# jason-li-831202/Vehicle-CV-ADAS

Measured on AMD Instinct MI355X. Metric: frames/sec end-to-end (detect+lane+NMS+track) per GPU; conv MFMA util %, higher is better.
Workload: dtype fp16x3

## Files before the change

### include/adas_hip.h

```cpp
#ifndef ADAS_HIP_H
#define ADAS_HIP_H
#include <stddef.h>
#include <stdint.h>

#ifdef __cplusplus
extern "C" {
#endif

typedef enum {
    ADAS_OK = 0,
    ADAS_ERR_INVALID = -1,
    ADAS_ERR_IO = -2,
    ADAS_ERR_FORMAT = -3,
    ADAS_ERR_HIP = -4,
    ADAS_ERR_CAPACITY = -5,
    ADAS_ERR_NO_DEVICE = -6
} adas_status;

const char* adas_last_error(void);
int adas_version(void);
int adas_device_count(void);
int adas_set_device(int index);
int adas_device_pci_bus_id(int index, char* out, int out_len);
int adas_malloc(void** d_ptr, size_t bytes);
// ... 5 lines not shown
int adas_host_free(void* h_ptr);
typedef struct adas_timer adas_timer;
int adas_timer_create(adas_timer** out);
int adas_timer_destroy(adas_timer* t);
int adas_timer_start(adas_timer* t, void* stream);
int adas_timer_stop(adas_timer* t, void* stream);
int adas_timer_elapsed_ms(adas_timer* t, float* ms);

typedef struct adas_engine adas_engine;

#define ADAS_PREC_BF16 0
#define ADAS_PREC_FP32 1
#define ADAS_PREC_FP16 2
#define ADAS_PREC_FP16X3 3

int adas_engine_create(const char* model_path, int precision, int max_batch, adas_engine** out);
int adas_engine_destroy(adas_engine* e);
int adas_engine_input_shape(const adas_engine* e, int64_t dims[4]);
int adas_engine_num_outputs(const adas_engine* e);
int adas_engine_output_shape(const adas_engine* e, int index, int64_t dims[4], int* ndim);
const char* adas_engine_output_name(const adas_engine* e, int index);
int adas_engine_infer_host(adas_engine* e, const float* h_input_nchw, int batch, float* const* h_outputs);
int adas_engine_infer_device(adas_engine* e, const float* d_input_nchw, int batch, void* stream);
int adas_engine_accepts_packed_input(const adas_engine* e);
int adas_engine_precision(const adas_engine* e);
int adas_engine_model_io_half(const adas_engine* e);
int adas_engine_infer_device_packed(adas_engine* e, const uint16_t* d_input_nhwc4, int batch, void* stream);
const float* adas_engine_output_device(const adas_engine* e, int index);
int adas_engine_stats(const adas_engine* e, double* flops_per_frame, double* weight_bytes, int* num_layers);
int adas_engine_profile(adas_engine* e, const float* d_input_nchw, int batch, int iters, float* ms_per_layer,
                        int max_layers, int* num_layers);
int adas_engine_detect_sink_supported(const adas_engine* e);
int adas_engine_detect_sink_shape(const adas_engine* e, int32_t* layout, int32_t* num_anchors, int32_t* num_classes);
int adas_engine_set_detect_sink(adas_engine* e, float* d_best_conf, int32_t* d_best_cls);
int adas_engine_layer_info(const adas_engine* e, int layer, char* name, int name_cap, double* flops, int* kind);
int adas_engine_layer_kernel(const adas_engine* e, int layer, int batch, char* name, int name_cap);
int adas_engine_prepare(adas_engine* e, int batch);
int adas_engine_ml_info(const adas_engine* e, int batch, int32_t* n_launches, int32_t* n_layers, int32_t* n_items);
int adas_engine_ml_status(const adas_engine* e, int batch, uint32_t* error_word);
int adas_engine_launch_count(adas_engine* e, int batch);
int adas_engine_ml_counters(const adas_engine* e, int batch, int launch, uint32_t head16[16]);
typedef struct adas_ml_view {
    uint64_t buf;
    int32_t cs, coff, c, h, w;
} adas_ml_view;
typedef struct adas_ml_layer_desc {
    int32_t kernel, stride, act, res_mode, up_c, halo_bn;
    adas_ml_view x, y, res, up;
} adas_ml_layer_desc;
int adas_debug_ml_plan(const adas_ml_layer_desc* layers, int n_layers, int batch, int precision, int32_t* deps, int32_t* targets,
                       uint64_t* items, int items_cap, int32_t summary[4]);
int adas_debug_conv_route(const adas_ml_layer_desc* layer, int batch, int precision, char* name, int name_cap);
int adas_debug_h8x3_onepass(const adas_ml_layer_desc* layer, int batch);
#define ADAS_PLAN_COLS 29
int adas_engine_plan(const adas_engine* e, int64_t* rows, int rows_cap, int32_t* n_ops, uint64_t* weight_bytes);
int adas_debug_engine_plan(const void* tables, size_t bytes, int precision, int max_batch, int64_t* rows, int rows_cap, int32_t* n_ops,
                           uint64_t* weight_bytes);
#define ADAS_LABEL_CAP 96
int adas_engine_schedule(const adas_engine* e, int batch, int32_t* step_of, int32_t* role, int cap, int32_t* n_ops, int32_t* n_steps);
int adas_debug_engine_schedule(const void* tables, size_t bytes, int precision, int max_batch, int batch, int32_t* step_of, int32_t* role,
                               char* labels, int cap, int32_t* n_ops, int32_t* n_steps);
int adas_engine_fetch_activation(adas_engine* e, int layer, int batch, float* h_out_nchw, int64_t dims[4]);

int adas_preprocess_yolo(const uint8_t* d_frames_bgr, int n, int src_h, int src_w, float* d_out_nchw, int dst_h,
                         int dst_w, int keep_ratio, void* stream);
int adas_preprocess_ufld(const uint8_t* d_frames_bgr, int n, int src_h, int src_w, float* d_out_nchw, int in_h,
                         int in_w, double crop_ratio, void* stream);
int adas_preprocess_yolo_packed(const uint8_t* d_frames_bgr, int n, int src_h, int src_w, uint16_t* d_out_nhwc4, int dst_h,
                                int dst_w, int keep_ratio, void* stream);
int adas_preprocess_ufld_packed(const uint8_t* d_frames_bgr, int n, int src_h, int src_w, uint16_t* d_out_nhwc4, int in_h,
                                int in_w, double crop_ratio, void* stream);
int adas_preprocess_yolo_packed_prec(const uint8_t* d_frames_bgr, int n, int src_h, int src_w, uint16_t* d_out_nhwc4, int dst_h,
                                     int dst_w, int keep_ratio, int precision, void* stream);
int adas_preprocess_ufld_packed_prec(const uint8_t* d_frames_bgr, int n, int src_h, int src_w, uint16_t* d_out_nhwc4, int in_h,
                                     int in_w, double crop_ratio, int precision, void* stream);

typedef struct adas_yolo_post adas_yolo_post;

#define ADAS_HEAD_V8 0
#define ADAS_HEAD_V5 1
#define ADAS_HEAD_V5_LITE 2
#define ADAS_NMS_REFERENCE 0
#define ADAS_NMS_GREEDY 1

typedef struct {
    int32_t layout;
    int32_t num_anchors;
    int32_t num_classes;
    int32_t nms_mode;
    double box_score;
    double iou_thr;
    int32_t pad_h, pad_w;
    double ratio_h, ratio_w;
    int32_t max_candidates;
    int32_t reserved;
} adas_yolo_post_params;

int adas_letterbox_params(int src_h, int src_w, int dst_h, int dst_w, int keep_ratio, adas_yolo_post_params* p);

int adas_yolo_post_create(const adas_yolo_post_params* p, int max_batch, adas_yolo_post** out);
int adas_yolo_post_destroy(adas_yolo_post* h);
int adas_yolo_post_set_input_size(adas_yolo_post* h, int in_h, int in_w);
int adas_yolo_post_run(adas_yolo_post* h, const float* d_head, int batch, void* stream);
int adas_yolo_post_scan_views(adas_yolo_post* h, float** d_best_conf, int32_t** d_best_cls);
int adas_yolo_post_run_prescanned(adas_yolo_post* h, const float* d_head, int batch, void* stream);
int adas_yolo_post_profile(adas_yolo_post* h, const float* d_head, int batch, int iters, float ms[2]);
// ... 490 lines not shown
```

### vehicle-cv-adas_amd/_lib.py

```python
import ctypes as C
import os

import numpy as np

HERE = os.path.dirname(os.path.abspath(__file__))
LIB_PATH = os.environ.get("ADAS_LIB") or os.path.join(HERE, "libadas_hip.so")

UFLD_MAX_POINTS = 128
HEAD_V8, HEAD_V5, HEAD_V5_LITE = 0, 1, 2
NMS_REFERENCE, NMS_GREEDY = 0, 1
PREC_BF16, PREC_FP32, PREC_FP16, PREC_FP16X3 = 0, 1, 2, 3
PRECISIONS = {"bf16": PREC_BF16, "fp32": PREC_FP32, "fp16": PREC_FP16, "fp16x3": PREC_FP16X3}


class AdasError(RuntimeError):
    def __init__(self, code, msg):
        super().__init__(f"libadas_hip error {code}: {msg}")
        self.code = code


class YoloPostParams(C.Structure):
    _fields_ = [("layout", C.c_int32), ("num_anchors", C.c_int32), ("num_classes", C.c_int32), ("nms_mode", C.c_int32),
                ("box_score", C.c_double), ("iou_thr", C.c_double), ("pad_h", C.c_int32), ("pad_w", C.c_int32),
                ("ratio_h", C.c_double), ("ratio_w", C.c_double), ("max_candidates", C.c_int32), ("reserved", C.c_int32)]
# ... 167 lines not shown


class MlView(C.Structure):
    _fields_ = [("buf", C.c_uint64), ("cs", C.c_int32), ("coff", C.c_int32), ("c", C.c_int32), ("h", C.c_int32), ("w", C.c_int32)]


class MlLayerDesc(C.Structure):
    _fields_ = [("kernel", C.c_int32), ("stride", C.c_int32), ("act", C.c_int32), ("res_mode", C.c_int32), ("up_c", C.c_int32), ("halo_bn", C.c_int32),
                ("x", MlView), ("y", MlView), ("res", MlView), ("up", MlView)]


TRACK_DTYPE = np.dtype([("tlwh", "f8", 4), ("score", "f8"), ("track_id", "i4"), ("state", "i4"), ("is_activated", "i4"),
                        ("class_id", "i4"), ("frame_id", "i4"), ("start_frame", "i4"), ("tracklet_len", "i4"), ("traj_len", "i4")])
TRAJECTORY_LEN = 30

_P = C.c_void_p
_SIGS = {
    "adas_last_error": (C.c_char_p, []),
    "adas_version": (C.c_int, []),
    "adas_device_count": (C.c_int, []),
    "adas_set_device": (C.c_int, [C.c_int]),
    "adas_device_pci_bus_id": (C.c_int, [C.c_int, C.c_char_p, C.c_int]),
    "adas_malloc": (C.c_int, [C.POINTER(_P), C.c_size_t]),
    "adas_free": (C.c_int, [_P]),
    "adas_memcpy_h2d": (C.c_int, [_P, _P, C.c_size_t]),
    "adas_memcpy_d2h": (C.c_int, [_P, _P, C.c_size_t]),
    "adas_synchronize": (C.c_int, []),
    "adas_host_alloc": (C.c_int, [C.POINTER(_P), C.c_size_t]),
    "adas_host_free": (C.c_int, [_P]),
    "adas_timer_create": (C.c_int, [C.POINTER(_P)]),
    "adas_timer_destroy": (C.c_int, [_P]),
    "adas_timer_start": (C.c_int, [_P, _P]),
    "adas_timer_stop": (C.c_int, [_P, _P]),
    "adas_timer_elapsed_ms": (C.c_int, [_P, C.POINTER(C.c_float)]),
    "adas_engine_create": (C.c_int, [C.c_char_p, C.c_int, C.c_int, C.POINTER(_P)]),
    "adas_engine_destroy": (C.c_int, [_P]),
    "adas_engine_input_shape": (C.c_int, [_P, C.POINTER(C.c_int64)]),
    "adas_engine_num_outputs": (C.c_int, [_P]),
    "adas_engine_output_shape": (C.c_int, [_P, C.c_int, C.POINTER(C.c_int64), C.POINTER(C.c_int)]),
    "adas_engine_output_name": (C.c_char_p, [_P, C.c_int]),
    "adas_engine_infer_host": (C.c_int, [_P, _P, C.c_int, C.POINTER(_P)]),
    "adas_engine_infer_device": (C.c_int, [_P, _P, C.c_int, _P]),
    "adas_engine_accepts_packed_input": (C.c_int, [_P]),
    "adas_engine_precision": (C.c_int, [_P]),
    "adas_engine_prepare": (C.c_int, [_P, C.c_int]),
    "adas_engine_ml_info": (C.c_int, [_P, C.c_int, C.POINTER(C.c_int32), C.POINTER(C.c_int32), C.POINTER(C.c_int32)]),
    "adas_engine_ml_status": (C.c_int, [_P, C.c_int, C.POINTER(C.c_uint32)]),
    "adas_engine_launch_count": (C.c_int, [_P, C.c_int]),
    "adas_engine_ml_counters": (C.c_int, [_P, C.c_int, C.c_int, C.POINTER(C.c_uint32)]),
    "adas_debug_ml_plan": (C.c_int, [C.POINTER(MlLayerDesc), C.c_int, C.c_int, C.c_int, C.POINTER(C.c_int32), C.POINTER(C.c_int32), C.POINTER(C.c_uint64),
                                     C.c_int, C.POINTER(C.c_int32)]),
    "adas_debug_conv_route": (C.c_int, [C.POINTER(MlLayerDesc), C.c_int, C.c_int, C.c_char_p, C.c_int]),
    "adas_debug_h8x3_onepass": (C.c_int, [C.POINTER(MlLayerDesc), C.c_int]),
    "adas_engine_plan": (C.c_int, [_P, C.POINTER(C.c_int64), C.c_int, C.POINTER(C.c_int32), C.POINTER(C.c_uint64)]),
    "adas_debug_engine_plan": (C.c_int, [C.c_char_p, C.c_size_t, C.c_int, C.c_int, C.POINTER(C.c_int64), C.c_int, C.POINTER(C.c_int32), C.POINTER(C.c_uint64)]),
    "adas_engine_schedule": (C.c_int, [_P, C.c_int, C.POINTER(C.c_int32), C.POINTER(C.c_int32), C.c_int, C.POINTER(C.c_int32), C.POINTER(C.c_int32)]),
    "adas_debug_engine_schedule": (C.c_int, [C.c_char_p, C.c_size_t, C.c_int, C.c_int, C.c_int, C.POINTER(C.c_int32), C.POINTER(C.c_int32), C.c_char_p,
                                             C.c_int, C.POINTER(C.c_int32), C.POINTER(C.c_int32)]),
    "adas_engine_model_io_half": (C.c_int, [_P]),
    "adas_engine_infer_device_packed": (C.c_int, [_P, _P, C.c_int, _P]),
    "adas_engine_output_device": (_P, [_P, C.c_int]),
    "adas_engine_stats": (C.c_int, [_P, C.POINTER(C.c_double), C.POINTER(C.c_double), C.POINTER(C.c_int)]),
    "adas_engine_profile": (C.c_int, [_P, _P, C.c_int, C.c_int, _P, C.c_int, C.POINTER(C.c_int)]),
    "adas_engine_layer_info": (C.c_int, [_P, C.c_int, C.c_char_p, C.c_int, C.POINTER(C.c_double), C.POINTER(C.c_int)]),
    "adas_engine_layer_kernel": (C.c_int, [_P, C.c_int, C.c_int, C.c_char_p, C.c_int]),
    "adas_engine_fetch_activation": (C.c_int, [_P, C.c_int, C.c_int, _P, C.POINTER(C.c_int64)]),
    "adas_preprocess_yolo": (C.c_int, [_P, C.c_int, C.c_int, C.c_int, _P, C.c_int, C.c_int, C.c_int, _P]),
    "adas_preprocess_ufld": (C.c_int, [_P, C.c_int, C.c_int, C.c_int, _P, C.c_int, C.c_int, C.c_double, _P]),
    "adas_preprocess_yolo_packed": (C.c_int, [_P, C.c_int, C.c_int, C.c_int, _P, C.c_int, C.c_int, C.c_int, _P]),
    "adas_preprocess_ufld_packed": (C.c_int, [_P, C.c_int, C.c_int, C.c_int, _P, C.c_int, C.c_int, C.c_double, _P]),
    "adas_preprocess_yolo_packed_prec": (C.c_int, [_P, C.c_int, C.c_int, C.c_int, _P, C.c_int, C.c_int, C.c_int, C.c_int, _P]),
    "adas_preprocess_ufld_packed_prec": (C.c_int, [_P, C.c_int, C.c_int, C.c_int, _P, C.c_int, C.c_int, C.c_double, C.c_int, _P]),
    "adas_letterbox_params": (C.c_int, [C.c_int, C.c_int, C.c_int, C.c_int, C.c_int, C.POINTER(YoloPostParams)]),
    "adas_yolo_post_create": (C.c_int, [C.POINTER(YoloPostParams), C.c_int, C.POINTER(_P)]),
    "adas_yolo_post_destroy": (C.c_int, [_P]),
    "adas_yolo_post_set_input_size": (C.c_int, [_P, C.c_int, C.c_int]),
    "adas_yolo_post_run": (C.c_int, [_P, _P, C.c_int, _P]),
    "adas_yolo_post_profile": (C.c_int, [_P, _P, C.c_int, C.c_int, C.POINTER(C.c_float)]),
    "adas_yolo_post_fetch": (C.c_int, [_P, C.c_int, C.POINTER(YoloCounts)] + [_P] * 9),
    "adas_yolo_post_fetch_dets": (C.c_int, [_P, C.c_int, C.POINTER(YoloCounts)] + [_P] * 5),
    "adas_yolo_post_device_views": (C.c_int, [_P] + [C.POINTER(_P)] * 4),
    "adas_yolo_post_scan_views": (C.c_int, [_P, C.POINTER(_P), C.POINTER(_P)]),
    "adas_yolo_post_run_prescanned": (C.c_int, [_P, _P, C.c_int, _P]),
    "adas_engine_detect_sink_supported": (C.c_int, [_P]),
    "adas_engine_detect_sink_shape": (C.c_int, [_P, C.POINTER(C.c_int32), C.POINTER(C.c_int32), C.POINTER(C.c_int32)]),
    "adas_engine_set_detect_sink": (C.c_int, [_P, _P, _P]),
    "adas_pipeline_detect_sink": (C.c_int, [_P]),
    "adas_yolo_post_capacity": (C.c_int, [_P, C.POINTER(C.c_int)]),
    "adas_yolo_post_head_shape": (C.c_int, [_P, C.POINTER(C.c_int32), C.POINTER(C.c_int32), C.POINTER(C.c_int32)]),
    "adas_effdet_post_create": (C.c_int, [C.POINTER(EffdetPostParams), C.c_int, C.POINTER(_P)]),
    "adas_effdet_post_destroy": (C.c_int, [_P]),
    "adas_effdet_post_run": (C.c_int, [_P, _P, _P, _P, _P, C.c_int, _P]),
    "adas_effdet_post_fetch": (C.c_int, [_P, C.c_int, C.POINTER(C.c_int32), _P, _P, _P, _P]),
    "adas_effdet_tail_create": (C.c_int, [C.POINTER(EffdetTailParams), C.c_int, C.POINTER(_P)]),
    "adas_effdet_tail_destroy": (C.c_int, [_P]),
    "adas_effdet_tail_run": (C.c_int, [_P, _P, _P, C.c_int, _P]),
    "adas_effdet_tail_fetch": (C.c_int, [_P, C.c_int, C.POINTER(C.c_int32), _P, _P, _P, C.POINTER(C.c_int32)]),
    "adas_effdet_tail_device_views": (C.c_int, [_P, C.POINTER(_P), C.POINTER(_P), C.POINTER(_P), C.POINTER(_P)]),
    "adas_preprocess_effdet": (C.c_int, [_P, C.c_int, C.c_int, C.c_int, _P, C.c_int, C.c_int, C.c_int, _P]),
    "adas_ufld_decode_create": (C.c_int, [C.POINTER(UfldParams), C.c_int, C.POINTER(_P)]),
    "adas_ufld_decode_destroy": (C.c_int, [_P]),
    "adas_ufld_decode_run": (C.c_int, [_P, _P, _P, _P, _P, C.c_size_t, C.c_size_t, C.c_size_t, C.c_size_t, C.c_int, _P]),
    "adas_ufld_decode_fetch": (C.c_int, [_P, C.c_int, _P, _P, _P]),
    "adas_ufld_decode_upload": (C.c_int, [_P, C.c_int, _P, _P, _P]),
    "adas_ufld1_decode_create": (C.c_int, [C.POINTER(Ufld1Params), C.c_int, C.POINTER(_P)]),
    "adas_ufld1_decode_set_source_size": (C.c_int, [_P, C.c_int, C.c_int]),
# ... 229 lines not shown
```

### vehicle-cv-adas_amd/csrc/conv_pw_x3.hip

```cpp
#include "kernels.h"
#include "elem16.h"
#include <stdlib.h>

namespace adas {

typedef __attribute__((ext_vector_type(4))) float wf32x4;
typedef __attribute__((ext_vector_type(4))) uint32_t wu32x4;

__device__ __forceinline__ float pwx_act(float v, int act) {
    if (act == ACT_SILU) return x3_silu(v);
    if (act == ACT_RELU) return fmaxf(v, 0.0f);
    if (act == ACT_LEAKY) return fmaxf(v, 0.1f * v);
    return v;
}

__device__ __forceinline__ void pwx_store(void* out, size_t o, const float v[4], int out_f32) {
    if (out_f32) *reinterpret_cast<float4*>((float*)out + o) = make_float4(v[0], v[1], v[2], v[3]);
    else x3_store4((x3s*)out + o, v);
}

struct PwxDev {
    const x3s* in;
    const uint16_t* wfrag;
    const float* bias;
    void* out;
    int in_cs, in_coff, cin;
    int out_cs, out_coff, cout, out_f32;
    int M;
    int stride, Wo, HoWo, W, HW;
    int act;
    int NT, NTL, mtiles;
    const x3s* up;
    int up_cs, up_coff, up_ks, up_W, up_HW;
};

template <int KS, bool TAIL>
__global__ __launch_bounds__(512) void conv_pwx3_kernel(PwxDev a) {
    Fp16::enter();
    extern __shared__ __attribute__((aligned(16))) uint16_t wl[];
    const int tid = threadIdx.x, lane = tid & 63, wave = tid >> 6;
    const int lrow = lane & 15, kg = lane >> 4;
    const int nt0 = blockIdx.y * a.NTL;
    const int ntl = a.NT - nt0 < a.NTL ? a.NT - nt0 : a.NTL;
    float* bl = reinterpret_cast<float*>(wl + (size_t)a.NTL * KS * 1024);
    {
        const int n16 = ntl * KS * 128;
        const uint16_t* wsrc = a.wfrag + (size_t)nt0 * KS * 1024;
        stage_lds16<512, 8>(wl, wsrc, n16, tid);
        for (int i = tid; i < ntl * 16; i += 512) bl[i] = a.bias[nt0 * 16 + i];
    }
    __syncthreads();
    const int tail_valid = a.cin - (KS - 1) * 32;
    const bool tail_zero = TAIL && kg * 8 >= tail_valid;

    for (int mt = blockIdx.x * 8 + wave; mt < a.mtiles; mt += gridDim.x * 8) {
        const int m = mt * 16 + lrow;
        const bool ok = m < a.M;
        const int mm = ok ? m : 0;
        size_t ipix;
        if (a.stride == 1) {
            ipix = (size_t)mm;
        } else {
            const int n = mm / a.HoWo, rem = mm - n * a.HoWo;
            const int oy = rem / a.Wo, ox = rem - oy * a.Wo;
            ipix = (size_t)n * a.HW + (size_t)(oy * a.stride) * a.W + ox * a.stride;
        }
        const wu32x4* ip = reinterpret_cast<const wu32x4*>(a.in + ipix * a.in_cs + a.in_coff + kg * 8);
        wu32x4 xh[KS], xl[KS];
        if (a.up) {
            const int n = mm / a.HW, rem = mm - n * a.HW;
            const int oy = rem / a.W, ox = rem - oy * a.W;
            const wu32x4* up = reinterpret_cast<const wu32x4*>(a.up + ((size_t)n * a.up_HW + (size_t)(oy >> 1) * a.up_W + (ox >> 1)) * a.up_cs + a.up_coff + kg * 8);
#pragma unroll
            for (int ks = 0; ks < KS; ++ks) {
                if (ks < a.up_ks) {
                    xh[ks] = up[ks * 8];
                    xl[ks] = up[ks * 8 + 1];
                } else {
                    xh[ks] = __builtin_nontemporal_load(ip + ks * 8);
                    xl[ks] = __builtin_nontemporal_load(ip + ks * 8 + 1);
                }
            }
        } else {
#pragma unroll
            for (int ks = 0; ks < KS; ++ks) {
                xh[ks] = __builtin_nontemporal_load(ip + ks * 8);
                xl[ks] = __builtin_nontemporal_load(ip + ks * 8 + 1);
            }
        }
        if (tail_zero) {
            xh[KS - 1] = wu32x4{0u, 0u, 0u, 0u};
            xl[KS - 1] = wu32x4{0u, 0u, 0u, 0u};
        }

        const size_t obase = (size_t)mm * a.out_cs + a.out_coff + kg * 4 + nt0 * 16;
        for (int nt = 0; nt < ntl; ++nt) {
            wf32x4 accm{0.f, 0.f, 0.f, 0.f}, accx{0.f, 0.f, 0.f, 0.f};
#pragma unroll
            for (int ks = 0; ks < KS; ++ks) {
                const uint16_t* wp = wl + ((size_t)(nt * KS + ks) * 128 + lane) * 8;
                const wu32x4 wh = *reinterpret_cast<const wu32x4*>(wp);
                const wu32x4 wlo = *reinterpret_cast<const wu32x4*>(wp + 512);
                accm = Fp16::mfma(wh, xh[ks], accm);
                accx = Fp16::mfma(wh, xl[ks], accx);
                accx = Fp16::mfma(wlo, xh[ks], accx);
            }
            const int c = nt * 16 + kg * 4;
            if (!ok || nt0 * 16 + c >= a.cout) continue;
            const float4 b4 = *reinterpret_cast<const float4*>(bl + c);
            const float bb[4] = {b4.x, b4.y, b4.z, b4.w};
            float v[4];
#pragma unroll
            for (int r = 0; r < 4; ++r) v[r] = pwx_act((accm[r] + accx[r] * kX3Down) + bb[r], a.act);
            pwx_store(a.out, obase + nt * 16, v, a.out_f32);
        }
    }
}

static const int PWX_MAX_LDS = 150 * 1024;

static int pwx_max_split() {
    static int v = -1;
    if (v < 0) {
        const char* e = getenv("ADAS_PWX3_MAXSPLIT");
        v = e ? atoi(e) : 4;
        if (v < 0) v = 0;
        if (v > 8) v = 8;
    }
    return v;
}
static int pwx_tiles_per_wg(int nt, int ks) {
    for (int split = 1; split <= pwx_max_split(); ++split) {
        const int ntl = (nt + split - 1) / split;
        if ((size_t)ntl * ks * 2048 + (size_t)ntl * 64 <= (size_t)PWX_MAX_LDS) return ntl;
    }
    return 0;
}

bool pw_x3_applicable(int kh, int kw, int stride, int pad, int res_mode, const TView& in, const TView& out) {
    if (in.f32) return false;
    if (kh != 1 || kw != 1 || pad != 0 || (stride != 1 && stride != 2) || res_mode != RES_NONE) return false;
    if (in.h == 1 && in.w == 1) return false;
    if ((in.c & 7) || (in.cs & 7) || (in.coff & 7) || (out.c & 3) || (out.cs & 3) || (out.coff & 3)) return false;
    if (!out.f32 && ((out.c & 7) || (out.cs & 7) || (out.coff & 7))) return false;
    const int ks = (in.c + 31) / 32, nt = (out.c + 15) / 16;
    if (!(ks <= 6 || ks == 8 || ks == 10 || ks == 12 || ks == 16)) return false;
    return pwx_tiles_per_wg(nt, ks) > 0;
}

template <int KS>
static hipError_t pwx_launch(const PwxDev& d, bool tail, dim3 grid, size_t lds, hipStream_t st) {
    static bool attr_done = false;
    if (!attr_done) {
        (void)hipFuncSetAttribute((const void*)conv_pwx3_kernel<KS, false>, hipFuncAttributeMaxDynamicSharedMemorySize, PWX_MAX_LDS);
        (void)hipFuncSetAttribute((const void*)conv_pwx3_kernel<KS, true>, hipFuncAttributeMaxDynamicSharedMemorySize, PWX_MAX_LDS);
        attr_done = true;
    }
    if (tail) hipLaunchKernelGGL((conv_pwx3_kernel<KS, true>), grid, dim3(512), lds, st, d);
    else hipLaunchKernelGGL((conv_pwx3_kernel<KS, false>), grid, dim3(512), lds, st, d);
    return hipGetLastError();
}

hipError_t launch_conv_pw_x3(const ConvArgs& a, hipStream_t st) {
    PwxDev d;
    d.in = (const x3s*)a.in.p; d.wfrag = (const uint16_t*)a.wgt; d.bias = a.bias; d.out = a.out.p;
    d.in_cs = a.in.cs; d.in_coff = a.in.coff; d.cin = a.in.c;
    d.out_cs = a.out.cs; d.out_coff = a.out.coff; d.cout = a.out.c; d.out_f32 = a.out.f32;
    d.M = a.m; d.stride = a.stride; d.Wo = a.out.w; d.HoWo = a.out.h * a.out.w; d.W = a.in.w; d.HW = a.in.h * a.in.w;
    d.act = a.act;
    d.up = nullptr; d.up_cs = d.up_coff = d.up_ks = d.up_W = d.up_HW = 0;
    if (a.up_c > 0) {
        if (a.stride != 1 || (a.up_c & 31) || a.up.c != a.up_c || 2 * a.up.h != a.in.h || 2 * a.up.w != a.in.w || a.up.f32 || ((a.up.cs | a.up.coff) & 7)) return hipErrorInvalidValue;
        d.up = (const x3s*)a.up.p; d.up_cs = a.up.cs; d.up_coff = a.up.coff; d.up_ks = a.up_c / 32; d.up_W = a.up.w; d.up_HW = a.up.h * a.up.w;
    }
    const int ks = (a.in.c + 31) / 32;
    d.NT = (a.out.c + 15) / 16;
    d.mtiles = (a.m + 15) / 16;
    d.NTL = pwx_tiles_per_wg(d.NT, ks);
    if (d.NTL <= 0) return hipErrorNotSupported;
    const int nsplit = (d.NT + d.NTL - 1) / d.NTL;
    const size_t lds = (size_t)d.NTL * ks * 2048 + (size_t)d.NTL * 64;
    int per_cu = (int)((160 * 1024) / (lds > 4096 ? lds : 4096));
    if (per_cu > 4) per_cu = 4;
    if (per_cu < 1) per_cu = 1;
    int gx = 256 * per_cu / nsplit;
    if (gx < 1) gx = 1;
    const int need = (d.mtiles + 7) / 8;
    if (gx > need) gx = need;
    const dim3 grid(gx, nsplit);
    const bool tail = (a.in.c & 31) != 0;
    switch (ks) {
        case 1: return pwx_launch<1>(d, tail, grid, lds, st);
        case 2: return pwx_launch<2>(d, tail, grid, lds, st);
        case 3: return pwx_launch<3>(d, tail, grid, lds, st);
        case 4: return pwx_launch<4>(d, tail, grid, lds, st);
        case 5: return pwx_launch<5>(d, tail, grid, lds, st);
        case 6: return pwx_launch<6>(d, tail, grid, lds, st);
        case 8: return pwx_launch<8>(d, tail, grid, lds, st);
        case 10: return pwx_launch<10>(d, tail, grid, lds, st);
        case 12: return pwx_launch<12>(d, tail, grid, lds, st);
        case 16: return pwx_launch<16>(d, tail, grid, lds, st);
    }
    return hipErrorInvalidValue;
}

struct FcxDev {
    const x3s* x;
    const uint16_t* w;
    const float* bias;
    void* out;
    int x_cs, x_coff, out_cs, out_coff;
    int batch, cout, kpad, act, out_f32;
};

template <int TN, int TM, int KS, int U>
__global__ __launch_bounds__(64 * KS) void fc_x3_kernel(FcxDev a) {
    Fp16::enter();
    const int tid = threadIdx.x, lane = tid & 63, wave = tid >> 6;
    const int lrow = lane & 15, kg = lane >> 4;
    const int n0 = blockIdx.x * (TN * 16);
    const int KT = a.kpad >> 5;
    const int ks0 = (int)((long)KT * wave / KS), ks1 = (int)((long)KT * (wave + 1) / KS);
    const int n = ks1 - ks0;

    const wu32x4* wp[TN];
#pragma unroll
    for (int i = 0; i < TN; ++i) wp[i] = reinterpret_cast<const wu32x4*>(a.w) + ((size_t)(blockIdx.x * TN + i) * KT + ks0) * 128 + lane;
    const wu32x4* xp[TM];
#pragma unroll
    for (int j = 0; j < TM; ++j) {
        const int m = j * 16 + lrow;
        xp[j] = reinterpret_cast<const wu32x4*>(a.x + (size_t)(m < a.batch ? m : 0) * a.x_cs + a.x_coff + kg * 8 + ks0 * 32);
    }

    wf32x4 accm[TN][TM], accx[TN][TM];
#pragma unroll
    for (int i = 0; i < TN; ++i)
#pragma unroll
        for (int j = 0; j < TM; ++j) {
            accm[i][j] = wf32x4{0.f, 0.f, 0.f, 0.f};
            accx[i][j] = wf32x4{0.f, 0.f, 0.f, 0.f};
        }
// ... 183 lines not shown
```

### vehicle-cv-adas_amd/csrc/engine.cpp

```cpp
#include "engine.h"
#include <string.h>
#include <string>
#include <vector>

using namespace adas;

int adas::free_engine(adas_engine* e) {
    if (!e) return ADAS_OK;
    for (auto& kv : e->schedules) free_schedule(&kv.second);
    e->schedules.clear();
    for (auto& b : e->bufs)
        if (b.d && b.alias_of < 0) (void)hipFree(b.d);
    if (e->d_weights) (void)hipFree(e->d_weights);
    if (e->d_input) (void)hipFree(e->d_input);
    for (auto& ev : e->events)
        if (ev) (void)hipEventDestroy(ev);
    delete e;
    return ADAS_OK;
}

extern "C" {

int adas_engine_destroy(adas_engine* e) { return free_engine(e); }

// ... 341 lines not shown
    a.k = a.kh * a.kw * a.in.c; a.kpad = (a.kh * a.kw * ((a.in.c + 31) / 32 * 32) + 31) / 32 * 32; a.m = batch * a.out.h * a.out.w; a.max_n = batch; a.prec = precision;
    a.halo_bn = d.halo_bn;
    if (d.up_c > 0) { a.up = view(d.up); a.up_c = d.up_c; }
    return a;
}

int adas_debug_ml_plan(const adas_ml_layer_desc* layers, int n_layers, int batch, int precision, int32_t* deps, int32_t* targets, uint64_t* items,
                       int items_cap, int32_t summary[4]) {
    ADAS_REQUIRE(layers && n_layers > 0 && batch > 0 && deps && targets && summary, ADAS_ERR_INVALID, "adas_debug_ml_plan: bad argument");
    std::vector<ConvArgs> ls;
    std::vector<int> ks;
    for (int i = 0; i < n_layers; ++i) {
        ls.push_back(conv_args_of_desc(layers[i], batch, precision));
        ks.push_back(layers[i].kernel);
    }
    std::string why;
    MlPlanInfo info;
    MlPlan* pl = ml_plan_create(ls, ks, precision, &why, &info, true);
    ADAS_REQUIRE(pl, ADAS_ERR_INVALID, "adas_debug_ml_plan: %s", why.c_str());
    ml_plan_destroy(pl);
    for (int i = 0; i < n_layers; ++i)
        for (int k = 0; k < ML_MAX_DEPS; ++k) {
            deps[i * ML_MAX_DEPS + k] = k < (int)info.deps[i].size() ? info.deps[i][k] : -1;
            targets[i * ML_MAX_DEPS + k] = k < (int)info.targets[i].size() ? info.targets[i][k] : 0;
        }
    summary[0] = info.n_items; summary[1] = info.grid; summary[2] = (int32_t)info.lds; summary[3] = info.order;
    if (items) {
        ADAS_REQUIRE(items_cap >= info.n_items, ADAS_ERR_CAPACITY, "adas_debug_ml_plan: %d items, room for %d", info.n_items, items_cap);
        for (int k = 0; k < info.n_items; ++k) items[k] = info.item_words[k];
    }
    return ADAS_OK;
}

int adas_debug_conv_route(const adas_ml_layer_desc* layer, int batch, int precision, char* name, int name_cap) {
    ADAS_REQUIRE(layer && batch > 0 && precision >= PREC_BF16 && precision <= PREC_X3 && name && name_cap > 0, ADAS_ERR_INVALID,
                 "adas_debug_conv_route: bad argument");
    ConvArgs a = conv_args_of_desc(*layer, batch, precision);
    const ConvPlan pl = plan_conv(precision, a.kh, a.kw, a.stride, a.pad, a.max_n, a.res_mode, a.in, a.out);
    a.kpad = pl.kpad;
    if (wants_x3h8_packing(precision, pl.kernel, a.kh, a.kw, a.stride, a.pad, a.res_mode, a.in, a.out)) a.wgt_h8x3 = (const void*)(uintptr_t)0x1000;
    snprintf(name, name_cap, "%s", conv_kernel_name(a));
    return ADAS_OK;
}

int adas_debug_h8x3_onepass(const adas_ml_layer_desc* layer, int batch) {
    if (!layer || batch <= 0) return -1;
    ConvArgs a = conv_args_of_desc(*layer, batch, PREC_X3);
    const ConvPlan pl = plan_conv(PREC_X3, a.kh, a.kw, a.stride, a.pad, a.max_n, a.res_mode, a.in, a.out);
    a.kpad = pl.kpad;
    if (wants_x3h8_packing(PREC_X3, pl.kernel, a.kh, a.kw, a.stride, a.pad, a.res_mode, a.in, a.out)) a.wgt_h8x3 = (const void*)(uintptr_t)0x1000;
    return (conv_route(a) == ConvRoute::H8X3 && halo8_x3_onepass(a)) ? 1 : 0;
}

int adas_engine_precision(const adas_engine* e) { return e ? e->prec : -1; }
int adas_engine_model_io_half(const adas_engine* e) { return e ? (int)((e->hdr.in_cpad >> 16) & 1u) : 0; }

int adas_engine_accepts_packed_input(const adas_engine* e) {
    return (e && e->prec != PREC_X3 && e->ops.size() >= 2 && e->ops[0].skip && e->ops[1].kernel == CONV_STEM) ? 1 : 0;
}

int adas_engine_infer_device_packed(adas_engine* e, const uint16_t* d_input_nhwc4, int batch, void* stream) {
    ADAS_REQUIRE(e && d_input_nhwc4 && batch > 0 && batch <= e->max_batch, ADAS_ERR_INVALID, "adas_engine_infer_device_packed: bad argument");
    ADAS_REQUIRE(adas_engine_accepts_packed_input(e), ADAS_ERR_INVALID,
                 "this engine's first layer is not the fused stem (fp32 mode or ADAS_NO_STEM): feed the fp32 NCHW tensor instead");
    e->last = (hipStream_t)stream;
    return engine_forward(e, reinterpret_cast<const float*>(d_input_nhwc4), batch, (hipStream_t)stream, true);
}

const float* adas_engine_output_device(const adas_engine* e, int index) {
    if (!e || index < 0 || index >= (int)e->outs.size()) return nullptr;
    const EngOut& o = e->outs[index];
    return (const float*)e->bufs[o.buf].d + o.offset;
}

int adas_engine_infer_host(adas_engine* e, const float* h_input, int batch, float* const* h_outputs) {
    ADAS_REQUIRE(e && h_input && h_outputs && batch > 0 && batch <= e->max_batch, ADAS_ERR_INVALID, "adas_engine_infer_host: bad argument");
    size_t in_bytes = (size_t)batch * e->hdr.in_c * e->hdr.in_h * e->hdr.in_w * 4;
    ADAS_HIP_TRY(hipMemcpyAsync(e->d_input, h_input, in_bytes, hipMemcpyHostToDevice, 0));
    int rc = adas_engine_infer_device(e, e->d_input, batch, nullptr);
    if (rc != ADAS_OK) return rc;
    for (size_t i = 0; i < e->outs.size(); ++i) {
        const EngOut& o = e->outs[i];
        const EngBuf& b = e->bufs[o.buf];
        size_t frame_stride = (size_t)b.h * b.w * b.c;
        ADAS_HIP_TRY(hipMemcpy2DAsync(h_outputs[i], o.elems * 4, (const float*)b.d + o.offset, frame_stride * 4, o.elems * 4, batch,
                                      hipMemcpyDeviceToHost, 0));
    }
    ADAS_HIP_TRY(hipStreamSynchronize(0));
    if (e->mode == adas_engine::ML) {
        uint32_t w = 0;
        int rc = adas_engine_ml_status(e, batch, &w);
        if (rc != ADAS_OK) return rc;
    }
    return ADAS_OK;
}

int adas_engine_profile(adas_engine* e, const float* d_input, int batch, int iters, float* ms_per_layer, int max_layers, int* num_layers) {
    ADAS_REQUIRE(e && d_input && batch > 0 && batch <= e->max_batch && iters > 0 && ms_per_layer, ADAS_ERR_INVALID, "adas_engine_profile: bad argument");
    const int n = (int)e->ops.size();
    ADAS_REQUIRE(max_layers >= n, ADAS_ERR_INVALID, "need room for %d layers", n);
    {
        int rc = engine_prepare(e, batch);
        if (rc != ADAS_OK) return rc;
    }
    const std::vector<Step>& steps = e->schedules.at(batch).steps;
    const size_t n_ev = (steps.size() > 8 ? steps.size() : 8) + 1;
// ... 71 lines not shown
```

### vehicle-cv-adas_amd/csrc/kernels.h

```cpp
#pragma once
#include <hip/hip_runtime.h>
#include <stdint.h>

namespace adas {

enum { PREC_BF16 = 0, PREC_FP32 = 1, PREC_FP16 = 2, PREC_X3 = 3 };
inline bool prec_is16(int prec) { return prec == PREC_BF16 || prec == PREC_FP16; }
inline int prec_esize(int prec) { return prec_is16(prec) ? 2 : 4; }
enum { ACT_NONE = 0, ACT_SILU = 1, ACT_RELU = 2, ACT_LEAKY = 3 ,
       ACT_HSWISH = 4 , ACT_HSIGMOID = 5 , ACT_RELU6 = 6  };
enum { RES_NONE = 0, RES_AFTER_ACT = 1, RES_BEFORE_ACT = 2 };

int persist_slots(int which);

struct TView {
    void* p;
    int cs, coff, c;
    int h, w;
    int f32;
};

struct ConvArgs {
    TView in, out, res;
    const void* wgt;
// ... 88 lines not shown
bool depth2space_supported(const TView& in, const TView& out);
hipError_t launch_depth2space(TView in, TView out, int n, int prec, hipStream_t st);
hipError_t launch_detect_v6(const TView* ins, float* out, int n, int nc, int A, const int strides[3], hipStream_t st);
hipError_t launch_detect_v6_dfl(const TView* ins, float* out, int n, int nc, int A, const int strides[3], hipStream_t st);
bool sppf_pool3_applicable(int prec, const TView& in, const TView out[3]);
hipError_t launch_sppf_pool3(const TView& in, const TView out[3], int n, int prec, hipStream_t st);
hipError_t launch_detect_v8(const TView* ins, float* out, int n, int nc, int A, const int strides[3], hipStream_t st);
hipError_t launch_detect_v8_fused(const TView* hidden, const void* const* wfrag, const float* const* bias, float* out, int n, int nc, int A,
                                  const int strides[3], int prec, hipStream_t st, float* sink_conf = nullptr, int* sink_cls = nullptr);
hipError_t launch_detect_v8_fused_x3(const TView* hidden, const void* const* wfrag, const float* const* bias, int kt_box, int kt_cls, float* out, int n, int nc,
                                     int A, const int strides[3], hipStream_t st_, float* sink_conf = nullptr, int* sink_cls = nullptr);
bool det5_applicable(int prec, int nc, const TView& in, const TView& logits);
size_t det5_weight_bytes(int no, int cin);
hipError_t launch_pack_weights_det5(const float* src, void* dst, int no, int cin, int prec, hipStream_t st);
hipError_t launch_detect_v5_fused(const TView* hidden, const void* const* wfrag, const float* const* bias, float* out, int n, int nc, int A,
                                  const int strides[3], const float* d_anchors, int prec, hipStream_t st, float* sink_conf = nullptr, int* sink_cls = nullptr);
hipError_t launch_detect_v5(const TView* ins, float* out, int n, int nc, int A, const int strides[3],
                            const float* d_anchors, hipStream_t st);
hipError_t launch_layernorm(const float* in, void* out, const float* gamma, const float* beta, int n, int len, float eps,
                            int prec, hipStream_t st);
hipError_t launch_pack_weights(const float* src, void* dst, int cout, int cout_pad, int taps, int cin, int cin_pad, int kpad,
                               int prec, hipStream_t st);
bool stem_applicable(int prec, int in_c_true, int kh, int kw, int stride, int pad, int act, int res_mode, const TView& out, bool pool,
                     const TView& pool_out);
size_t stem_weight_bytes(int kh, int cout);
size_t stem2_weight_bytes();
void stem2_pack_weights(const float* w_ohwi_32x3x3x16, uint16_t* dst_host, int prec);
bool stem2_applicable(int prec, int kh, int pad, int act, const TView& stem_out, int kh2, int kw2, int stride2, int pad2, int act2, int res_mode2,
                      const TView& out2);
hipError_t launch_conv_stem2(const float* nchw, int n, int c_true, int H, int W, int kh, int pad, const void* wfrag, const float* bias,
                             const TView& stem_out, const void* wfrag2, const float* bias2, const TView& out2, bool packed_in, int prec, hipStream_t st);
void stem_pack_weights(const float* w_ohwi, int cout, int kh, int kw, int cs, int c_true, uint16_t* dst_host, int prec);
bool stem_x3_applicable(int in_c_true, int kh, int kw, int stride, int pad, int act, int res_mode, const TView& out);
size_t stem_x3_weight_bytes(int kh, int cout);
void stem_x3_pack_weights(const float* w_ohwi, int cout, int kh, int kw, int cs, int c_true, uint16_t* dst_host);
hipError_t launch_conv_stem_x3(const float* nchw, int n, int c_true, int H, int W, int kh, int pad, int act, const void* wfrag, const float* bias,
                               const TView& out, hipStream_t st);
bool stem2_x3_applicable(int in_c_true, int kh, int pad, int act, const TView& stem_out, int kh2, int kw2, int stride2, int pad2, int act2, int res_mode2,
                         const TView& out2);
size_t stem2_x3_weight_bytes();
void stem2_x3_pack_weights(const float* w_ohwi_32x3x3x16, uint16_t* dst_host);
hipError_t launch_conv_stem2_x3(const float* nchw, int n, int c_true, int H, int W, int kh, int pad, const void* wfrag, const float* bias,
                                const TView& stem_out, const void* wfrag2, const float* bias2, const TView& out2, hipStream_t st);
bool stem_pool_x3_applicable(int in_c_true, int kh, int kw, int stride, int pad, int act, int res_mode, const TView& conv_out, const TView& pool_out);
hipError_t launch_conv_stem_pool_x3(const float* nchw, int n, int c_true, int H, int W, int pad, const void* wfrag, const float* bias,
                                    const TView& conv_out, const TView& pool_out, hipStream_t st);
hipError_t launch_conv_stem(const float* nchw, int n, int c_true, int H, int W, int kh, int pad, int act, const void* wfrag,
                            const float* bias, const TView& conv_out, bool pool, const TView& pool_out, bool packed_in, int prec, hipStream_t st);
inline int halo_bn(int cout) { return cout <= 16 ? 16 : (cout <= 32 ? 32 : ((cout > 64 && cout <= 96) ? 48 : 64)); }
int plan_halo_bn(int max_n, int stride, const TView& in, const TView& out);
hipError_t launch_pack_weights_halo(const float* src, void* dst, int cout, int cout_pad, int cin, int cin_pad, int prec, hipStream_t st, int bn = 0);
bool pw_x3_applicable(int kh, int kw, int stride, int pad, int res_mode, const TView& in, const TView& out);
hipError_t launch_conv_pw_x3(const ConvArgs& a, hipStream_t st);
bool fc_x3_applicable(int kh, int kw, int stride, const TView& in, const TView& out);
hipError_t launch_fc_x3(const ConvArgs& a, hipStream_t st);
hipError_t launch_pack_weights_fcx3(const float* src, void* dst, int cout, int cout_pad, int cin, int kpad, hipStream_t st);
hipError_t launch_pack_weights_fc(const float* src, void* dst, int cout, int cout_pad, int cin, int kpad, int prec, hipStream_t st);
bool se_gate_supported(const TView& in, const TView& gate, int cr, uint64_t w_elems, uint64_t b_elems);
hipError_t launch_se_gate(const TView& in, const TView& gate, const float* w1, const float* w2, int cr, int act_hidden, int act_gate, int n, int prec, hipStream_t st,
                          const TView* scratch = nullptr);
bool scale_supported(const TView& in, const TView& gate, const TView& out);
hipError_t launch_scale(const TView& in, const TView& gate, const TView& out, int n, int prec, hipStream_t st);
bool shuffle_supported(const TView& in, const TView& out, int groups);
hipError_t launch_shuffle(const TView& in, const TView& out, int groups, int n, int prec, hipStream_t st);
bool wsum_supported(int n_in, const TView* ins, const TView& out);
hipError_t launch_wsum(int n_in, const TView* ins, const float* w, const TView& out, int n, int act, int prec, hipStream_t st);
bool dwconv_supported(int k, int stride, int pad, int res_mode, const TView& in, const TView& out);
hipError_t launch_dwconv(const TView& in, const TView& out, const TView& res, int res_mode, const float* wgt, const float* bias, int n, int k,
                         int stride, int pad, int act, int prec, hipStream_t st);
bool attention_supported(int nh, int kd, int hd, const TView& qkv, const TView& out);
hipError_t launch_attention(const TView& qkv, const TView& out, int n, int nh, int kd, int hd, float scale, int prec, hipStream_t st);
hipError_t launch_nhwc_to_nchw(TView in, float* out, int n, int prec, hipStream_t st);

}
```

Measured before the change: 5660.

## Add K-streaming pointwise fp16x3 conv kernel with async LDS pipelining

Adds a new pointwise fp16x3 conv body that streams the K dimension. Activation and weight chunks are loaded with buffer_load_lds into a 2-3 slot ring buffer, and a persistent grid walks over M passes. The old body keeps all weights for a column split resident in LDS. The new body is chosen by default when that old plan would split the output channels or use more than 80KB of LDS and there are enough passes. The aim is to stop reloading activations once per output-channel split and to raise occupancy, at the cost of re-streaming weights for every pass and adding more barriers.

```diff
diff --git a/include/adas_hip.h b/include/adas_hip.h
--- a/include/adas_hip.h
+++ b/include/adas_hip.h
@@ -81,6 +81,8 @@
                        uint64_t* items, int items_cap, int32_t summary[4]);
 int adas_debug_conv_route(const adas_ml_layer_desc* layer, int batch, int precision, char* name, int name_cap);
 int adas_debug_h8x3_onepass(const adas_ml_layer_desc* layer, int batch);
+int adas_debug_pwx3_body(int mode);
+int adas_debug_pwx3_plan(int cin, int cout, int m, int stride, int out[4]);
 #define ADAS_PLAN_COLS 29
 int adas_engine_plan(const adas_engine* e, int64_t* rows, int rows_cap, int32_t* n_ops, uint64_t* weight_bytes);
 int adas_debug_engine_plan(const void* tables, size_t bytes, int precision, int max_batch, int64_t* rows, int rows_cap, int32_t* n_ops,
diff --git a/vehicle-cv-adas_amd/_lib.py b/vehicle-cv-adas_amd/_lib.py
--- a/vehicle-cv-adas_amd/_lib.py
+++ b/vehicle-cv-adas_amd/_lib.py
@@ -243,6 +243,8 @@
                                      C.c_int, C.POINTER(C.c_int32)]),
     "adas_debug_conv_route": (C.c_int, [C.POINTER(MlLayerDesc), C.c_int, C.c_int, C.c_char_p, C.c_int]),
     "adas_debug_h8x3_onepass": (C.c_int, [C.POINTER(MlLayerDesc), C.c_int]),
+    "adas_debug_pwx3_body": (C.c_int, [C.c_int]),
+    "adas_debug_pwx3_plan": (C.c_int, [C.c_int, C.c_int, C.c_int, C.c_int, C.POINTER(C.c_int)]),
     "adas_engine_plan": (C.c_int, [_P, C.POINTER(C.c_int64), C.c_int, C.POINTER(C.c_int32), C.POINTER(C.c_uint64)]),
     "adas_debug_engine_plan": (C.c_int, [C.c_char_p, C.c_size_t, C.c_int, C.c_int, C.POINTER(C.c_int64), C.c_int, C.POINTER(C.c_int32), C.POINTER(C.c_uint64)]),
     "adas_engine_schedule": (C.c_int, [_P, C.c_int, C.POINTER(C.c_int32), C.POINTER(C.c_int32), C.c_int, C.POINTER(C.c_int32), C.POINTER(C.c_int32)]),
diff --git a/vehicle-cv-adas_amd/csrc/conv_pw_x3.hip b/vehicle-cv-adas_amd/csrc/conv_pw_x3.hip
--- a/vehicle-cv-adas_amd/csrc/conv_pw_x3.hip
+++ b/vehicle-cv-adas_amd/csrc/conv_pw_x3.hip
@@ -1,6 +1,7 @@
 #include "kernels.h"
 #include "elem16.h"
 #include <stdlib.h>
+#include <atomic>
 
 namespace adas {
 
@@ -32,6 +33,8 @@
     int NT, NTL, mtiles;
     const x3s* up;
     int up_cs, up_coff, up_ks, up_W, up_HW;
+    uint32_t in_bytes, up_bytes, wgt_bytes;
+    int npass;
 };
 
 template <int KS, bool TAIL>
@@ -117,6 +120,169 @@
     }
 }
 
+constexpr uint32_t PWK_OOB = 0xF0000000u;
+constexpr int PWK_MIN_PASSES = 128;
+typedef __attribute__((address_space(3))) void* pwk_lds_vp;
+
+template <int N>
+__device__ __forceinline__ void pwk_wait_vm() {
+    asm volatile("s_waitcnt vmcnt(%0) lgkmcnt(0)" ::"n"(N) : "memory");
+}
+
+template <int NTG, int G>
+struct PwkGeom {
+    static constexpr int PT = 2, NPT = (8 / G) * PT;
+    static constexpr int ACT_B = NPT * 2048, WGT_B = G * NTG * 2048, SLOT = ACT_B + WGT_B, BIAS_B = 2048;
+    static constexpr int NS = 3 * SLOT + BIAS_B <= 160 * 1024 ? 3 : 2;
+    static constexpr int APW = NPT * 2 / 8, WPW = G * NTG * 2 / 8, PPW = APW + WPW;
+    static constexpr int LDS = NS * SLOT + BIAS_B;
+};
+
+template <int KS, int NTG, int G>
+__global__ __launch_bounds__(512) void conv_pwx3_kstream_kernel(PwxDev a) {
+    using Gm = PwkGeom<NTG, G>;
+    constexpr int PT = Gm::PT, NPT = Gm::NPT, NS = Gm::NS, APW = Gm::APW, WPW = Gm::WPW, SLOT = Gm::SLOT, ACT_B = Gm::ACT_B;
+    Fp16::enter();
+    extern __shared__ __attribute__((aligned(16))) uint16_t wl[];
+    unsigned char* lds8 = reinterpret_cast<unsigned char*>(wl);
+    const int tid = threadIdx.x, lane = tid & 63, wave = __builtin_amdgcn_readfirstlane(tid >> 6);
+    const int lrow = lane & 15, kg = lane >> 4;
+    const int g = wave % G, s = wave / G;
+    const int t0 = g * a.NTL;
+    const int nmine = a.NT - t0 < a.NTL ? (a.NT - t0 > 0 ? a.NT - t0 : 0) : a.NTL;
+    float* bl = reinterpret_cast<float*>(lds8 + NS * SLOT);
+    for (int i = tid; i < a.NT * 16; i += 512) bl[i] = a.bias[i];
+    __syncthreads();
+    const int tail_valid = a.cin - (KS - 1) * 32;
+    const bool tail_zero = kg * 8 >= tail_valid;
+
+    __amdgpu_buffer_rsrc_t rin = __builtin_amdgcn_make_buffer_rsrc((void*)a.in, 0, a.in_bytes, 0x00020000);
+    __amdgpu_buffer_rsrc_t rup = __builtin_amdgcn_make_buffer_rsrc((void*)(a.up ? a.up : a.in), 0, a.up ? a.up_bytes : a.in_bytes, 0x00020000);
+    __amdgpu_buffer_rsrc_t rwg = __builtin_amdgcn_make_buffer_rsrc((void*)a.wfrag, 0, a.wgt_bytes, 0x00020000);
+
+    uint32_t wvo[8];
+#pragma unroll
+    for (int i = 0; i < WPW; ++i) {
+        const int p = wave + 8 * i, tile = p >> 1;
+        wvo[i] = tile < a.NT ? (uint32_t)((tile * KS * 2 + (p & 1)) * 1024 + lane * 16) : PWK_OOB;
+    }
+    uint32_t avo[2], uvo[2];
+    auto pass_offsets = [&](int P) {
+#pragma unroll
+        for (int i = 0; i < APW; ++i) {
+            const int q = wave + 8 * i;
+            const int m = (P * NPT + (q >> 1)) * 16 + lrow;
+            const int mm = m < a.M ? m : 0;
+            size_t ipix;
+            if (a.stride == 1) {
+                ipix = (size_t)mm;
+            } else {
+                const int n = mm / a.HoWo, rem = mm - n * a.HoWo;
+                const int oy = rem / a.Wo, ox = rem - oy * a.Wo;
+                ipix = (size_t)n * a.HW + (size_t)(oy * a.stride) * a.W + ox * a.stride;
+            }
+            const uint32_t sub = (uint32_t)(kg * 32 + (q & 1) * 16);
+            avo[i] = P < a.npass ? (uint32_t)((ipix * a.in_cs + a.in_coff) * 4) + sub : PWK_OOB;
+            uvo[i] = PWK_OOB;
+            if (a.up && P < a.npass) {
+                const int n = mm / a.HW, rem = mm - n * a.HW;
+                const int oy = rem / a.W, ox = rem - oy * a.W;
+                uvo[i] = (uint32_t)((((size_t)n * a.up_HW + (size_t)(oy >> 1) * a.up_W + (ox >> 1)) * a.up_cs + a.up_coff) * 4) + sub;
+            }
+        }
+    };
+    int Pi = blockIdx.x, ksi = 0, sloti = 0;
+    auto issue = [&]() {
+        unsigned char* sb = lds8 + sloti * SLOT;
+        if (ksi < a.up_ks) {
+#pragma unroll
+            for (int i = 0; i < APW; ++i)
+                __builtin_amdgcn_raw_ptr_buffer_load_lds(rup, (pwk_lds_vp)(sb + (wave + 8 * i) * 1024), 16, uvo[i], ksi * 128, 0, 0);
+        } else {
+#pragma unroll
+            for (int i = 0; i < APW; ++i)
+                __builtin_amdgcn_raw_ptr_buffer_load_lds(rin, (pwk_lds_vp)(sb + (wave + 8 * i) * 1024), 16, avo[i], ksi * 128, 0, 0);
+        }
+        const bool live = Pi < a.npass;
+#pragma unroll
+        for (int i = 0; i < WPW; ++i)
+            __builtin_amdgcn_raw_ptr_buffer_load_lds(rwg, (pwk_lds_vp)(sb + ACT_B + (wave + 8 * i) * 1024), 16, live ? wvo[i] : PWK_OOB, ksi * 2048, 0, 0);
+        sloti = sloti + 1 == NS ? 0 : sloti + 1;
+        if (++ksi == KS) {
+            ksi = 0;
+            Pi += gridDim.x;
+            pass_offsets(Pi);
+        }
+    };
+    pass_offsets(Pi);
+#pragma unroll
+    for (int u = 0; u < NS - 1; ++u) issue();
+
+    int slot = 0;
+    for (int P = blockIdx.x; P < a.npass; P += gridDim.x) {
+        wf32x4 accm[PT][NTG], accx[PT][NTG];
+#pragma unroll
+        for (int p = 0; p < PT; ++p)
+#pragma unroll
+            for (int j = 0; j < NTG; ++j) {
+                accm[p][j] = wf32x4{0.f, 0.f, 0.f, 0.f};
+                accx[p][j] = wf32x4{0.f, 0.f, 0.f, 0.f};
+            }
+#pragma unroll 1
+        for (int ks = 0; ks < KS; ++ks) {
+            pwk_wait_vm<(NS - 2) * Gm::PPW>();
+            __builtin_amdgcn_sched_barrier(0);
+            __builtin_amdgcn_s_barrier();
+            __builtin_amdgcn_sched_barrier(0);
+            issue();
+            __builtin_amdgcn_sched_barrier(0);
+            const unsigned char* sb = lds8 + slot * SLOT;
+            wu32x4 xh[PT], xl[PT];
+#pragma unroll
+            for (int p = 0; p < PT; ++p) {
+                const unsigned char* xp = sb + ((s * PT + p) * 2) * 1024 + lane * 16;
+                xh[p] = *reinterpret_cast<const wu32x4*>(xp);
+                xl[p] = *reinterpret_cast<const wu32x4*>(xp + 1024);
+                if (ks == KS - 1 && tail_zero) {
+                    xh[p] = wu32x4{0u, 0u, 0u, 0u};
+                    xl[p] = wu32x4{0u, 0u, 0u, 0u};
+                }
+            }
+#pragma unroll
+            for (int j = 0; j < NTG; ++j) {
+                const unsigned char* wp = sb + ACT_B + (t0 + j) * 2048 + lane * 16;
+                const wu32x4 wh = *reinterpret_cast<const wu32x4*>(wp);
+                const wu32x4 wlo = *reinterpret_cast<const wu32x4*>(wp + 1024);
+#pragma unroll
+                for (int p = 0; p < PT; ++p) {
+                    accm[p][j] = Fp16::mfma(wh, xh[p], accm[p][j]);
+                    accx[p][j] = Fp16::mfma(wh, xl[p], accx[p][j]);
+                    accx[p][j] = Fp16::mfma(wlo, xh[p], accx[p][j]);
+                }
+            }
+            slot = slot + 1 == NS ? 0 : slot + 1;
+        }
+#pragma unroll
+        for (int p = 0; p < PT; ++p) {
+            const int m = (P * NPT + s * PT + p) * 16 + lrow;
+            if (m >= a.M) continue;
+            const size_t obase = (size_t)m * a.out_cs + a.out_coff + kg * 4;
+#pragma unroll
+            for (int j = 0; j < NTG; ++j) {
+                const int c = (t0 + j) * 16 + kg * 4;
+                if (j >= nmine || c >= a.cout) continue;
+                const float4 b4 = *reinterpret_cast<const float4*>(bl + c);
+                const float bb[4] = {b4.x, b4.y, b4.z, b4.w};
+                float v[4];
+#pragma unroll
+                for (int r = 0; r < 4; ++r) v[r] = pwx_act((accm[p][j][r] + accx[p][j][r] * kX3Down) + bb[r], a.act);
+                pwx_store(a.out, obase + (t0 + j) * 16, v, a.out_f32);
+            }
+        }
+    }
+    pwk_wait_vm<0>();
+}
+
 static const int PWX_MAX_LDS = 150 * 1024;
 
 static int pwx_max_split() {
@@ -159,6 +325,69 @@
     if (tail) hipLaunchKernelGGL((conv_pwx3_kernel<KS, true>), grid, dim3(512), lds, st, d);
     else hipLaunchKernelGGL((conv_pwx3_kernel<KS, false>), grid, dim3(512), lds, st, d);
     return hipGetLastError();
+}
+
+template <int KS, int NTG, int G>
+static hipError_t pwk_launch_one(const PwxDev& d, int gx, hipStream_t st) {
+    constexpr int lds = PwkGeom<NTG, G>::LDS;
+    static bool attr_done = false;
+    if (!attr_done) {
+        (void)hipFuncSetAttribute((const void*)conv_pwx3_kstream_kernel<KS, NTG, G>, hipFuncAttributeMaxDynamicSharedMemorySize, lds);
+        attr_done = true;
+    }
+    hipLaunchKernelGGL((conv_pwx3_kstream_kernel<KS, NTG, G>), dim3(gx), dim3(512), lds, st, d);
+    return hipGetLastError();
+}
+template <int KS>
+static hipError_t pwk_launch(const PwxDev& d, const Pwx3Plan& pl, hipStream_t st) {
+    if (pl.g == 4) return pwk_launch_one<KS, 8, 4>(d, pl.wgs, st);
+    return pl.ntg_cap == 4 ? pwk_launch_one<KS, 4, 2>(d, pl.wgs, st) : pwk_launch_one<KS, 8, 2>(d, pl.wgs, st);
+}
+
+static std::atomic<int> g_pwx3_mode{0};
+int pwx3_body_mode(int mode) {
+    if (mode < 0 || mode > 2) return g_pwx3_mode.load();
+    return g_pwx3_mode.exchange(mode);
+}
+
+static bool pwk_ks_ok(int ks) { return ks == 4 || ks == 5 || ks == 6 || ks == 8 || ks == 10 || ks == 12 || ks == 16; }
+
+bool pwx3_plan(int cin, int cout, int m, int stride, int mode, Pwx3Plan* pl) {
+    if (cin <= 0 || cout <= 0 || m <= 0 || (stride != 1 && stride != 2) || (cin & 7)) return false;
+    const int ks = (cin + 31) / 32, nt = (cout + 15) / 16, mtiles = (m + 15) / 16;
+    if (!(ks <= 6 || ks == 8 || ks == 10 || ks == 12 || ks == 16)) return false;
+    const int ntl = pwx_tiles_per_wg(nt, ks);
+    if (ntl <= 0) return false;
+    Pwx3Plan r{};
+    r.body = 1;
+    r.ntl = ntl;
+    r.nsplit = (nt + ntl - 1) / ntl;
+    r.lds = (int)((size_t)ntl * ks * 2048 + (size_t)ntl * 64);
+    int per_cu = (160 * 1024) / (r.lds > 4096 ? r.lds : 4096);
+    if (per_cu > 4) per_cu = 4;
+    if (per_cu < 1) per_cu = 1;
+    int gx = 256 * per_cu / r.nsplit;
+    if (gx < 1) gx = 1;
+    const int need = (mtiles + 7) / 8;
+    if (gx > need) gx = need;
+    r.gx = gx;
+    r.wgs = gx * r.nsplit;
+    *pl = r;
+    if (mode == 1 || !pwk_ks_ok(ks) || nt > 32) return true;
+    Pwx3Plan k{};
+    k.body = 2;
+    k.nsplit = 1;
+    k.g = nt > 16 ? 4 : 2;
+    k.ntl = (nt + k.g - 1) / k.g;
+    k.ntg_cap = (k.g == 2 && k.ntl <= 4) ? 4 : 8;
+    const int npt = (8 / k.g) * 2;
+    k.npass = (mtiles + npt - 1) / npt;
+    k.lds = k.g == 4 ? PwkGeom<8, 4>::LDS : (k.ntg_cap == 4 ? PwkGeom<4, 2>::LDS : PwkGeom<8, 2>::LDS);
+    const int per_wg = (k.npass + 255) / 256;
+    k.gx = k.wgs = (k.npass + per_wg - 1) / per_wg;
+    const bool wants = r.nsplit > 1 || r.lds > 80 * 1024;
+    if (mode == 2 || (wants && k.npass >= PWK_MIN_PASSES)) *pl = k;
+    return true;
 }
 
 hipError_t launch_conv_pw_x3(const ConvArgs& a, hipStream_t st) {
@@ -176,18 +405,27 @@
     const int ks = (a.in.c + 31) / 32;
     d.NT = (a.out.c + 15) / 16;
     d.mtiles = (a.m + 15) / 16;
-    d.NTL = pwx_tiles_per_wg(d.NT, ks);
-    if (d.NTL <= 0) return hipErrorNotSupported;
-    const int nsplit = (d.NT + d.NTL - 1) / d.NTL;
-    const size_t lds = (size_t)d.NTL * ks * 2048 + (size_t)d.NTL * 64;
-    int per_cu = (int)((160 * 1024) / (lds > 4096 ? lds : 4096));
-    if (per_cu > 4) per_cu = 4;
-    if (per_cu < 1) per_cu = 1;
-    int gx = 256 * per_cu / nsplit;
-    if (gx < 1) gx = 1;
-    const int need = (d.mtiles + 7) / 8;
-    if (gx > need) gx = need;
-    const dim3 grid(gx, nsplit);
+    const size_t in_bytes = (size_t)a.n * a.in.h * a.in.w * a.in.cs * 4;
+    const size_t up_bytes = a.up_c > 0 ? (size_t)a.n * a.up.h * a.up.w * a.up.cs * 4 : 0;
+    const size_t lim = (size_t)1 << 31;
+    Pwx3Plan pl;
+    if (!pwx3_plan(a.in.c, a.out.c, a.m, a.stride, (in_bytes < lim && up_bytes < lim) ? g_pwx3_mode.load() : 1, &pl)) return hipErrorNotSupported;
+    d.NTL = pl.ntl;
+    d.in_bytes = (uint32_t)in_bytes; d.up_bytes = (uint32_t)up_bytes; d.wgt_bytes = (uint32_t)((size_t)d.NT * ks * 2048); d.npass = pl.npass;
+    if (pl.body == 2) {
+        switch (ks) {
+            case 4: return pwk_launch<4>(d, pl, st);
+            case 5: return pwk_launch<5>(d, pl, st);
+            case 6: return pwk_launch<6>(d, pl, st);
+            case 8: return pwk_launch<8>(d, pl, st);
+            case 10: return pwk_launch<10>(d, pl, st);
+            case 12: return pwk_launch<12>(d, pl, st);
+            case 16: return pwk_launch<16>(d, pl, st);
+        }
+        return hipErrorInvalidValue;
+    }
+    const size_t lds = (size_t)pl.lds;
+    const dim3 grid(pl.gx, pl.nsplit);
     const bool tail = (a.in.c & 31) != 0;
     switch (ks) {
         case 1: return pwx_launch<1>(d, tail, grid, lds, st);
diff --git a/vehicle-cv-adas_amd/csrc/engine.cpp b/vehicle-cv-adas_amd/csrc/engine.cpp
--- a/vehicle-cv-adas_amd/csrc/engine.cpp
+++ b/vehicle-cv-adas_amd/csrc/engine.cpp
@@ -417,6 +417,15 @@
     return (conv_route(a) == ConvRoute::H8X3 && halo8_x3_onepass(a)) ? 1 : 0;
 }
 
+int adas_debug_pwx3_body(int mode) { return pwx3_body_mode(mode); }
+
+int adas_debug_pwx3_plan(int cin, int cout, int m, int stride, int out[4]) {
+    Pwx3Plan pl;
+    if (!out || !pwx3_plan(cin, cout, m, stride, pwx3_body_mode(-1), &pl)) return -1;
+    out[0] = pl.body; out[1] = pl.nsplit; out[2] = pl.lds; out[3] = pl.wgs;
+    return 0;
+}
+
 int adas_engine_precision(const adas_engine* e) { return e ? e->prec : -1; }
 int adas_engine_model_io_half(const adas_engine* e) { return e ? (int)((e->hdr.in_cpad >> 16) & 1u) : 0; }
 
diff --git a/vehicle-cv-adas_amd/csrc/kernels.h b/vehicle-cv-adas_amd/csrc/kernels.h
--- a/vehicle-cv-adas_amd/csrc/kernels.h
+++ b/vehicle-cv-adas_amd/csrc/kernels.h
@@ -164,6 +164,13 @@
 hipError_t launch_pack_weights_halo(const float* src, void* dst, int cout, int cout_pad, int cin, int cin_pad, int prec, hipStream_t st, int bn = 0);
 bool pw_x3_applicable(int kh, int kw, int stride, int pad, int res_mode, const TView& in, const TView& out);
 hipError_t launch_conv_pw_x3(const ConvArgs& a, hipStream_t st);
+struct Pwx3Plan {
+    int body, nsplit, lds, wgs;
+    int gx, ntl;
+    int g, ntg_cap, npass;
+};
+bool pwx3_plan(int cin, int cout, int m, int stride, int mode, Pwx3Plan* pl);
+int pwx3_body_mode(int mode);
 bool fc_x3_applicable(int kh, int kw, int stride, const TView& in, const TView& out);
 hipError_t launch_fc_x3(const ConvArgs& a, hipStream_t st);
 hipError_t launch_pack_weights_fcx3(const float* src, void* dst, int cout, int cout_pad, int cin, int kpad, hipStream_t st);
```

After: 5647 (median of 2 runs). Within noise of the previous version (-0.2%).
